# CrystalAnalyst/Lsm

Measured on AMD Instinct MI355X. Metric: GiB/s device-resident SSTable block encode+decode, 4 KiB blocks, 1/2/4/8 GPU, higher is better.
Workload: dtype u8; 1 GPU; U: 1048576 blocks/GPU x block_size 4096, decode + re-encode (16-B uniform keys, 100-B values); blocks_per_gpu=1048576, entries_per_gpu=32474205, encoded_bytes_per_gpu=4226189427, decoded_bytes_per_gpu=4286595060, block_size=4096, segments_per_gpu=2045, parallelism=block-sharded x1 (no data-path collective), encode_output=segments packed (lsmblk_encode_batch), rccl_world=1

## Files before the change

### lsm_amd/csrc/lsmblk_gpu.hip

```cpp
#include "lsmblk_dev.hpp"

namespace {


struct DecodeArgs {
  const uint8_t* blocks;
  const uint64_t* blk_off;
  uint64_t nblk;
  uint8_t* keys;
  uint32_t* key_off;
  uint8_t* vals;
  uint32_t* val_off;
  uint64_t* ts;
  uint64_t entry_cap, key_cap, val_cap;
  uint64_t* stats;
  const uint32_t* agg;
  const uint64_t* tile_pre;
  uint32_t tail;
  uint64_t* blk_ent;
  uint32_t skip;
  uint64_t* bagg;
  uint64_t* bbase;
  uint64_t* tagg;
  uint64_t* tinc;
  uint64_t lag;
  uint64_t lag_bytes;
  uint64_t* dbg;
  uint32_t tag, poll;
};

constexpr uint32_t kTile = 64;
constexpr uint32_t kDbgTiles = 32768, kDbgWords = 16 + 8 * kDbgTiles;
__device__ __forceinline__ void dbg_trace(uint64_t* dbg, uint64_t t, uint32_t k) {
  if (kDiag && dbg && t < kDbgTiles && lane_id() == 0) dbg[16 + 8 * t + k] = __builtin_amdgcn_s_memrealtime();
}


constexpr uint32_t kLB = 2;
#ifndef LSMBLK_XEB
#define LSMBLK_XEB 4
#endif
constexpr uint32_t kEB = LSMBLK_XEB;
constexpr uint32_t kEBBlock = 2;


constexpr uint32_t kDecImg = 4128;
constexpr uint32_t kDecMaxE = 128;
constexpr uint32_t kDecOut = 4032;

struct alignas(16) DecLds {
  uint8_t img[kDecImg];
  alignas(16) uint8_t out[kDecOut];
};
static_assert(sizeof(DecLds) == 8160, "decode LDS: 20 blocks per CU");

struct DecTables {
  uint16_t epos[kDecMaxE], pfx[kDecMaxE], sfx[kDecMaxE];
  uint32_t kout[kDecMaxE + 1], vout[kDecMaxE + 1];
};
static_assert(sizeof(DecTables) <= kDecImg, "large-block tables overlay the image");

struct DecEnt {
  uint32_t epos, p, s, kout, vout, vl;
};

__device__ __forceinline__ void lds_read16(const uint8_t* base, uint32_t x, uint32_t (&v)[4]) {
  const u32x4 q = *reinterpret_cast<const u32x4*>(base + x);
  v[0] = q.x, v[1] = q.y, v[2] = q.z, v[3] = q.w;
}

constexpr int kLdAux = 0;

template <class Img>
__device__ void dec_simple_outputs(const DecodeArgs& a, const Img& im, const BlockHdr& h,
                                   uint64_t E0, uint64_t K0, uint64_t V0) {
  const uint32_t l = lane_id();
  uint64_t kc = 0, vc = 0;
  for (uint32_t c = 0; c < h.n; c += 64) {
    const uint32_t k = c + l;
    uint32_t off = 0, p = 0, s = 0, vl = 0;
    if (k < h.n) parse_entry(im, h, k, off, p, s, vl);
    const uint64_t kl = p + s;
    const uint64_t ki = wave_incl_scan<uint64_t>(kl), vi = wave_incl_scan<uint64_t>(vl);
    const uint64_t kpos = K0 + kc + ki - kl, vpos = V0 + vc + vi - vl;
    kc += __shfl(ki, 63, 64);
    vc += __shfl(vi, 63, 64);
    if (k < h.n) {
      const uint64_t e = E0 + k;
      if (e < a.entry_cap) {
        a.ts[e] = im.u64(off + 4 + s);
        a.key_off[e] = uint32_t(kpos);
        a.val_off[e] = uint32_t(vpos);
      }
      for (uint32_t t = 0; t < p; ++t)
        if (kpos + t < a.key_cap) a.keys[kpos + t] = uint8_t(im.u8(4 + t));
      for (uint32_t t = 0; t < s; ++t)
        if (kpos + p + t < a.key_cap) a.keys[kpos + p + t] = uint8_t(im.u8(off + 4 + t));
      for (uint32_t t = 0; t < vl; ++t)
        if (vpos + t < a.val_cap) a.vals[vpos + t] = uint8_t(im.u8(off + 14 + s + t));
    }
  }
}

__device__ __forceinline__ void st16(const rsrc_t& R, uint32_t off, const uint32_t (&v)[4]) {
  const u32x4 q = {v[0], v[1], v[2], v[3]};
  __builtin_amdgcn_raw_buffer_store_b128(q, R, off, 0, 0);
}

__device__ __forceinline__ void st_short(const rsrc_t& R, uint32_t off, uint32_t len, const uint32_t (&v)[4]) {
  if (len >= 8) {
    __builtin_amdgcn_raw_buffer_store_b64(u32x2{v[0], v[1]}, R, off, 0, 0);
    const uint32_t x = len - 8, sh = x & 3;
    const uint32_t w0 = x < 4 ? v[0] : v[1], w1 = x < 4 ? v[1] : v[2], w2 = x < 4 ? v[2] : v[3];
    __builtin_amdgcn_raw_buffer_store_b64(
        u32x2{__builtin_amdgcn_alignbyte(w1, w0, sh), __builtin_amdgcn_alignbyte(w2, w1, sh)}, R, off + x, 0, 0);
  } else if (len >= 4) {
    __builtin_amdgcn_raw_buffer_store_b32(v[0], R, off, 0, 0);
    __builtin_amdgcn_raw_buffer_store_b32(__builtin_amdgcn_alignbyte(v[1], v[0], len - 4), R, off + len - 4, 0, 0);
  } else {
    for (uint32_t i = 0; i < len; ++i)
      __builtin_amdgcn_raw_buffer_store_b8(uint8_t(v[0] >> (8 * i)), R, off + i, 0, 0);
  }
}

struct GlbSink {
  rsrc_t RK, RV;
  uint32_t kb, vb;
  __device__ __forceinline__ void put16(bool val, uint32_t off, const uint32_t (&v)[4]) const {
    st16(val ? RV : RK, (val ? vb : kb) + off, v);
  }
  __device__ __forceinline__ void put_short(bool val, uint32_t off, uint32_t len, const uint32_t (&v)[4]) const {
    st_short(val ? RV : RK, (val ? vb : kb) + off, len, v);
  }
};
struct LdsSink {
  uint8_t* out;
  uint32_t kb, vb;
  __device__ __forceinline__ void put16(bool val, uint32_t off, const uint32_t (&v)[4]) const {
    *reinterpret_cast<u32x4*>(out + (val ? vb : kb) + off) = u32x4{v[0], v[1], v[2], v[3]};
  }
  __device__ __forceinline__ void put_short(bool val, uint32_t off, uint32_t len, const uint32_t (&v)[4]) const {
    uint8_t* p = out + (val ? vb : kb) + off;
    if (len >= 8) {
      const uint32_t x = len - 8, sh = x & 3;
      const uint32_t w0 = x < 4 ? v[0] : v[1], w1 = x < 4 ? v[1] : v[2], w2 = x < 4 ? v[2] : v[3];
      *reinterpret_cast<u32x2*>(p) = u32x2{v[0], v[1]};
      *reinterpret_cast<u32x2*>(p + x) =
          u32x2{__builtin_amdgcn_alignbyte(w1, w0, sh), __builtin_amdgcn_alignbyte(w2, w1, sh)};
    } else if (len >= 4) {
      *reinterpret_cast<uint32_t*>(p) = v[0];
      *reinterpret_cast<uint32_t*>(p + len - 4) = __builtin_amdgcn_alignbyte(v[1], v[0], len - 4);
    } else {
      for (uint32_t i = 0; i < len; ++i) p[i] = uint8_t(v[0] >> (8 * i));
    }
  }
};

#ifndef LSMBLK_XDEC_VALN
#define LSMBLK_XDEC_VALN 1
#endif
template <class Sink>
__device__ __forceinline__ void dec_entry_runs(const DecodeArgs& a, DecLds& L, uint32_t lead, uint32_t n,
                                               const DecEnt (&ent)[2], uint64_t E0, uint64_t K0, uint64_t V0,
                                               const Sink& out, uint32_t skip) {
  const uint32_t l = lane_id();
  const uint8_t* img = L.img;
  const uint32_t fk = lead + 4;
#pragma unroll
  for (uint32_t it = 0; it < 2; ++it) {
    if (64 * it >= n) break;
    const uint32_t k = 64 * it + l;
    const bool live = k < n;
    const uint32_t epos = ent[it].epos, p = ent[it].p, s = ent[it].s;
    const uint32_t kout = ent[it].kout, vout = ent[it].vout, vl = ent[it].vl;
    const uint32_t sb = lead + epos + 4;
    const uint32_t kl = p + s;
    const bool kirr = live && (kl < 16 || sb < p);
    const bool kuni = !__ballot(kirr);
    const uint32_t nkmax = __builtin_amdgcn_readlane(wave_incl_max32(live ? (kl + 15) >> 4 : 0u), 63);
    const uint32_t nvmax = __builtin_amdgcn_readlane(wave_incl_max32(live && vl >= 16 ? (vl + 15) >> 4 : 0u), 63);
    const uint32_t vS = sb + s + 10, vD = out.vb + vout;
    bool valn = false;
    uint32_t vm = 0, vmmax = 0, vS1 = 0, vD1 = 0;
    if constexpr (std::is_same_v<Sink, LdsSink>) {
      valn = LSMBLK_XDEC_VALN && it == 0 && n <= 64 && !__ballot(live && (vl < 16 || (l == 0 && vS < (vD & 15)))) &&
             !(skip & (4 | 32 | 64));
      if (valn) {
        const uint32_t cs = l == 0 ? (vD >> 4) : ((vD + 15) >> 4), ce = (vD + vl - 1) >> 4;
        vm = live ? ce - cs + 1 : 0u;
        vmmax = __builtin_amdgcn_readlane(wave_incl_max32(vm), 63);
        vS1 = uint32_t(__shfl(int(vS), int(min(l + 1, 63u)), 64));
        vD1 = uint32_t(__shfl(int(vD), int(min(l + 1, 63u)), 64));
      }
    }
    if (!live) continue;
    if (!(skip & 8)) {
      const uint64_t e = E0 + k;
      const u32x2 q = LSMBLK_XALIGNED_LDS ? lds_qw_al(img, sb + s) : *reinterpret_cast<const u32x2*>(img + sb + s);
      a.ts[e] = __builtin_bswap64((uint64_t(q.y) << 32) | q.x);
      a.key_off[e] = uint32_t(K0 + kout);
      a.val_off[e] = uint32_t(V0 + vout);
    }
    if (!(skip & 2)) {
      auto merged = [&](uint32_t o, uint32_t (&v)[4]) {
        const u32x4 sq = *reinterpret_cast<const u32x4*>(img + sb + o - p);
        const u32x4 fq = *reinterpret_cast<const u32x4*>(img + fk + o);
        const uint32_t sv[4] = {sq.x, sq.y, sq.z, sq.w}, fv[4] = {fq.x, fq.y, fq.z, fq.w};
#pragma unroll
        for (uint32_t d = 0; d < 4; ++d) {
          const int32_t nf = int32_t(p) - int32_t(o + 4 * d);
          const uint32_t m = nf <= 0 ? 0u : nf >= 4 ? ~0u : (1u << (8 * nf)) - 1;
          v[d] = (fv[d] & m) | (sv[d] & ~m);
        }
      };
      if (kuni) {
        for (uint32_t t = 0; t < nkmax; ++t) {
          const uint32_t o = min(16 * t, kl - 16);
          uint32_t v[4];
          merged(o, v);
          out.put16(false, kout + o, v);
        }
      } else {
        for (uint32_t t = 0; t < kl; t += 16) {
          const uint32_t o = kl >= 16 ? min(t, kl - 16) : 0u;
          uint32_t v[4];
          if (sb + o >= p) {
            merged(o, v);
          } else {
#pragma unroll
            for (uint32_t d = 0; d < 4; ++d) {
              uint32_t wd = 0;
              for (uint32_t i = 0; i < 4; ++i) {
                const uint32_t x = o + 4 * d + i;
                wd |= uint32_t(x < p ? img[fk + x] : img[sb + x - p]) << (8 * i);
              }
              v[d] = wd;
            }
          }
          if (kl >= 16) out.put16(false, kout + o, v);
          else out.put_short(false, kout, kl, v);
        }
      }
    }
    if (valn) {
      uint8_t* const ob = L.out;
      auto funnel = [](const uint32_t (&d)[6], uint32_t x, uint32_t (&v)[4]) {
        const uint32_t m = (x & 4) ? ~0u : 0u;
        uint32_t y[5];
#pragma unroll
        for (uint32_t j = 0; j < 5; ++j) y[j] = __builtin_amdgcn_bitop3_b32(m, d[j + 1], d[j], 0xCA);
#pragma unroll
        for (uint32_t i = 0; i < 4; ++i) v[i] = __builtin_amdgcn_alignbyte(y[i + 1], y[i], x & 3);
      };
      auto rd8 = [&](uint32_t x, uint32_t& lo, uint32_t& hi) {
        const u32x2 q = *reinterpret_cast<const u32x2*>(img + x);
        lo = q.x, hi = q.y;
      };
      const uint32_t cs = l == 0 ? (vD >> 4) : ((vD + 15) >> 4);
      const uint32_t a0 = vS + 16 * cs - vD;
      uint32_t d[6], x8 = a0 & ~7u;
      rd8(x8, d[0], d[1]);
      rd8(x8 + 8, d[2], d[3]);
      rd8(x8 + 16, d[4], d[5]);
      for (uint32_t i = 0; i < vmmax; ++i) {
        if (i < vm) {
          uint32_t v[4];
          funnel(d, a0, v);
          const uint32_t c = cs + i, cut = vD + vl - 16 * c;
          if (cut < 16 && k + 1 < n) {
            const uint32_t a1 = vS1 + 16 * c - vD1, y8 = a1 & ~7u;
            uint32_t e[6], w[4];
            rd8(y8, e[0], e[1]);
            rd8(y8 + 8, e[2], e[3]);
            rd8(y8 + 16, e[4], e[5]);
            funnel(e, a1, w);
#pragma unroll
            for (uint32_t q = 0; q < 4; ++q) {
              const int32_t nb = int32_t(cut) - int32_t(4 * q);
              const uint32_t msk = nb <= 0 ? 0u : nb >= 4 ? ~0u : (1u << (8 * nb)) - 1;
              v[q] = (v[q] & msk) | (w[q] & ~msk);
            }
          }
          *reinterpret_cast<u32x4*>(ob + 16 * c) = u32x4{v[0], v[1], v[2], v[3]};
          d[0] = d[4], d[1] = d[5];
          x8 += 16;
          rd8(x8 + 8, d[2], d[3]);
          rd8(x8 + 16, d[4], d[5]);
        }
      }
    } else if (!(skip & 4)) {
      const uint32_t src = sb + s + 10;
      if (vl >= 16) {
        for (uint32_t i0 = 0; i0 < nvmax; i0 += kLB) {
          u32x4 q[kLB];
          uint32_t o[kLB];
          const uint32_t am = (skip & 32) ? 15u : (skip & 64) ? 3u : 0u;
#pragma unroll
          for (uint32_t j = 0; j < kLB; ++j) {
            o[j] = min(16 * (i0 + j), vl - 16);
            q[j] = *reinterpret_cast<const u32x4*>(img + ((src + o[j]) & ~am));
          }
#pragma unroll
          for (uint32_t j = 0; j < kLB; ++j) {
            const uint32_t v[4] = {q[j].x, q[j].y, q[j].z, q[j].w};
            const uint32_t xa = (out.vb + vout + o[j]) & ~am;
            out.put16(true, xa >= out.vb ? xa - out.vb : xa + am + 1 - out.vb, v);
          }
        }
      } else if (vl) {
        const u32x4 q = *reinterpret_cast<const u32x4*>(img + src);
        const uint32_t v[4] = {q.x, q.y, q.z, q.w};
        out.put_short(true, vout, vl, v);
      }
    }
  }
}

template <uint32_t B = kLB>
__device__ __forceinline__ void flush_run(uint8_t* gdst_aligned, const uint8_t* lds, uint32_t lo, uint32_t len) {
  flush_chunks<B, LSMBLK_XDEC_STORE>(gdst_aligned, lds, lo, len, lane_id(), 64);
}

template <uint32_t B>
__device__ __forceinline__ void flush_run_masked(uint8_t* gdst_aligned, const uint8_t* lds, uint32_t lo, uint32_t len) {
  const uint32_t end = lo + len, nc = (end + 15) >> 4;
  const uint32_t l = lane_id();
  for (uint32_t c0 = 0; c0 < nc; c0 += 64 * B) {
    u32x4 q[B];
#pragma unroll
    for (uint32_t j = 0; j < B; ++j) {
      const uint32_t c = c0 + 64 * j + l;
      if (c < nc) q[j] = *reinterpret_cast<const u32x4*>(lds + 16 * c);
    }
#pragma unroll
    for (uint32_t j = 0; j < B; ++j) {
      const uint32_t c = c0 + 64 * j + l;
      if (c < nc) {
        const uint32_t v[4] = {q[j].x, q[j].y, q[j].z, q[j].w};
        const uint32_t a0 = 16 * c < lo ? lo - 16 * c : 0u;
        const uint32_t a1 = min(end - 16 * c, 16u);
        store_chunk(gdst_aligned + 16 * c, v, a0, a1);
      }
    }
  }
}

__device__ void dec_fast_outputs(const DecodeArgs& a, DecLds& L, uint32_t lead, const BlockHdr& h,
                                 const DecEnt (&ent)[2], uint64_t E0, uint64_t K0, uint64_t V0, uint32_t K,
                                 uint32_t V, uint32_t skip) {
  const uint32_t kb = uint32_t(K0 & 15), vb = uint32_t(V0 & 15);
  const uint32_t vrun = (kb + K + 15) & ~15u;
  if (vrun + ((vb + V + 15) & ~15u) <= kDecOut) {
    dec_entry_runs(a, L, lead, h.n, ent, E0, K0, V0, LdsSink{L.out, kb, vrun + vb}, skip);
    wave_sync();
    flush_run(a.keys + (K0 - kb), L.out, kb, K);
    flush_run(a.vals + (V0 - vb), L.out + vrun, vb, V);
  } else {
    const GlbSink g{make_rsrc_exact(a.keys + (K0 - kb), kb + K), make_rsrc_exact(a.vals + (V0 - vb), vb + V), kb, vb};
    dec_entry_runs(a, L, lead, h.n, ent, E0, K0, V0, g, skip);
  }
}

constexpr uint32_t kBigB = 8;

__device__ __forceinline__ u32x4 gload16(const rsrc_t& R, uint32_t off) {
  return __builtin_amdgcn_raw_buffer_load_b128(R, off, 0, 0);
}

__device__ __forceinline__ void copy_run(const rsrc_t& RS, uint32_t so, uint32_t lim, const rsrc_t& RD, uint32_t dof,
                                         uint32_t len) {
  if (len == 0) return;
  if (len < 16) {
    uint32_t v[4] = {0, 0, 0, 0};
    if (so + 16 <= lim) {
      const u32x4 q = gload16(RS, so);
      v[0] = q.x, v[1] = q.y, v[2] = q.z, v[3] = q.w;
    } else {
      for (uint32_t i = 0; i < len; ++i) v[i >> 2] |= __builtin_amdgcn_raw_buffer_load_b8(RS, so + i, 0, 0) << (8 * (i & 3));
    }
    st_short(RD, dof, len, v);
    return;
  }
  const uint32_t np = (len + 15) >> 4, last = len - 16;
  for (uint32_t j0 = 0; j0 < np; j0 += kBigB) {
    u32x4 q[kBigB];
#pragma unroll
    for (uint32_t j = 0; j < kBigB; ++j)
      if (j0 + j < np) q[j] = gload16(RS, so + min(16 * (j0 + j), last));
#pragma unroll
    for (uint32_t j = 0; j < kBigB; ++j)
      if (j0 + j < np) {
        const uint32_t v[4] = {q[j].x, q[j].y, q[j].z, q[j].w};
        st16(RD, dof + min(16 * (j0 + j), last), v);
      }
  }
}

__device__ __forceinline__ void copy_run1(const rsrc_t& RS, uint32_t so, uint32_t lim, const rsrc_t& RD, uint32_t dof,
                                          uint32_t len) {
  if (len < 16) {
    copy_run(RS, so, lim, RD, dof, len);
    return;
  }
  const uint32_t last = len - 16;
  for (uint32_t o = 0;; o += 16) {
    const uint32_t x = min(o, last);
    const u32x4 q = gload16(RS, so + x);
    const uint32_t v[4] = {q.x, q.y, q.z, q.w};
    st16(RD, dof + x, v);
    if (x == last) break;
  }
}

constexpr uint32_t kCoop = 16;
__device__ __forceinline__ void copy_run_wave(const rsrc_t& RS, uint32_t so, const rsrc_t& RD, uint32_t dof,
                                              uint32_t len) {
  const uint32_t l = lane_id();
  const uint32_t np = (len + 15) >> 4, last = len - 16;
  for (uint32_t j0 = 0; j0 < np; j0 += 64 * kBigB) {
    u32x4 q[kBigB];
#pragma unroll
    for (uint32_t j = 0; j < kBigB; ++j) {
      const uint32_t idx = j0 + 64 * j + l;
      if (idx < np) q[j] = gload16(RS, so + min(16 * idx, last));
    }
#pragma unroll
    for (uint32_t j = 0; j < kBigB; ++j) {
      const uint32_t idx = j0 + 64 * j + l;
      if (idx < np) {
        const uint32_t v[4] = {q[j].x, q[j].y, q[j].z, q[j].w};
        st16(RD, dof + min(16 * idx, last), v);
      }
    }
  }
}

constexpr uint32_t kCopyScratch = 4 * 64 + 64;
static_assert(4 * kCopyScratch <= kDecOut, "the decode's large-block path lends its output image");

template <uint32_t B>
struct CopyBatch {
  u32x4 q[B];
  uint32_t dst[B];
};

template <uint32_t B>
__device__ __forceinline__ void copy_issue(const rsrc_t& RS, uint32_t g0, uint32_t total, uint32_t np, uint32_t first,
                                           uint32_t* sc, uint32_t& carry, CopyBatch<B>& c) {
  const uint32_t l = lane_id();
  const u32x4* rec = reinterpret_cast<const u32x4*>(sc);
  uint32_t* mark = sc + 4 * 64;
  uint32_t own[B];
#pragma unroll
  for (uint32_t j = 0; j < B; ++j) {
    const uint32_t G = g0 + 64 * j;
    own[j] = 0;
    if (G < total) {
      mark[l] = 0;
      wave_sync();
      if (np != 0 && first - G < 64u) mark[first - G] = l + 1;
      wave_sync();
      const uint32_t m = max(wave_incl_max32(mark[l]), carry);
      carry = __builtin_amdgcn_readlane(m, 63);
      own[j] = m - 1;
      wave_sync();
    }
  }
#pragma unroll
  for (uint32_t j = 0; j < B; ++j) {
    const uint32_t g = g0 + 64 * j + l;
    c.dst[j] = ~0u;
    if (g < total) {
      const u32x4 r = rec[own[j]];
      const uint32_t off = min(16 * (g - r.w), r.z);
      c.q[j] = gload16(RS, r.x + off);
      c.dst[j] = r.y + off;
    }
  }
}

template <uint32_t B>
__device__ __forceinline__ void copy_store(const rsrc_t& RD, const CopyBatch<B>& c) {
#pragma unroll
  for (uint32_t j = 0; j < B; ++j)
    if (c.dst[j] != ~0u) {
      const uint32_t v[4] = {c.q[j].x, c.q[j].y, c.q[j].z, c.q[j].w};
      st16(RD, c.dst[j], v);
    }
}

struct NoAfter {
  __device__ void operator()(uint32_t, uint32_t, uint32_t) const {}
};
template <uint32_t B = kBigB, class After = NoAfter>
__device__ __forceinline__ void copy_long_runs(bool longrun, const rsrc_t& RS, uint32_t so, const rsrc_t& RD,
                                               uint32_t dof, uint32_t len, uint32_t* sc, const After& after = After()) {
  const uint32_t l = lane_id();
  const uint32_t np = longrun ? (len + 15) >> 4 : 0u;
  const uint32_t incl = wave_incl_scan32(np);
  const uint32_t total = __builtin_amdgcn_readlane(incl, 63);
  const uint32_t first = incl - np;
  if (total == 0) {
    after(first, 0u, ~0u);
    return;
  }
  wave_sync();
  reinterpret_cast<u32x4*>(sc)[l] = u32x4{so, dof, len - 16, first};
  uint32_t carry = 0;
  for (uint32_t g0 = 0; g0 < total; g0 += 64 * B) {
    CopyBatch<B> c;
    copy_issue(RS, g0, total, np, first, sc, carry, c);
    copy_store(RD, c);
    after(first, g0, g0 + 64 * B >= total ? ~0u : g0 + 64 * B);
  }
}

__device__ __forceinline__ void dec_big_entry(const DecodeArgs& a, const DecTables& L, const GlbImg& im, uint32_t k,
                                              uint32_t lim, const rsrc_t& RK, uint32_t kb, uint64_t E0, uint64_t K0,
                                              uint64_t V0) {
  const rsrc_t& R = im.r;
  const uint32_t lead = im.lead, fk = lead + 4;
  const uint32_t epos = L.epos[k], p = L.pfx[k], s = L.sfx[k], kout = L.kout[k];
  const uint32_t sb = lead + epos + 4, kl = p + s;
  const uint64_t e = E0 + k;
  a.ts[e] = im.u64(epos + 4 + s);
  a.key_off[e] = uint32_t(K0 + kout);
  a.val_off[e] = uint32_t(V0 + L.vout[k]);
  for (uint32_t t = 0; t < kl; t += 16) {
    const uint32_t o = kl >= 16 ? min(t, kl - 16) : 0u;
    uint32_t v[4];
    if (sb + o >= p && sb + o - p + 16 <= lim && fk + o + 16 <= lim) {
      const u32x4 sq = gload16(R, sb + o - p), fq = gload16(R, fk + o);
      const uint32_t sv[4] = {sq.x, sq.y, sq.z, sq.w}, fv[4] = {fq.x, fq.y, fq.z, fq.w};
#pragma unroll
      for (uint32_t d = 0; d < 4; ++d) {
        const int32_t nf = int32_t(p) - int32_t(o + 4 * d);
        const uint32_t m = nf <= 0 ? 0u : nf >= 4 ? ~0u : (1u << (8 * nf)) - 1;
        v[d] = (fv[d] & m) | (sv[d] & ~m);
      }
    } else {
#pragma unroll
      for (uint32_t d = 0; d < 4; ++d) {
        uint32_t wd = 0;
        for (uint32_t i = 0; i < 4; ++i) {
          const uint32_t x = o + 4 * d + i;
          wd |= (x < p ? im.u8(4 + x) : im.u8(epos + 4 + x - p)) << (8 * i);
        }
        v[d] = wd;
      }
    }
    if (kl >= 16) st16(RK, kb + kout + o, v);
    else st_short(RK, kb + kout, kl, v);
  }
}

#ifndef LSMBLK_XDBB
#define LSMBLK_XDBB 8
#endif
constexpr uint32_t kDecBigB = LSMBLK_XDBB;

__device__ void dec_big_outputs(const DecodeArgs& a, const DecTables& L, const rsrc_t& R, uint32_t lead,
                                const BlockHdr& h, uint32_t n, uint64_t Eb, uint64_t K0, uint64_t V0, uint32_t K,
                                uint32_t V, uint32_t* sc) {
  const uint32_t l = lane_id();
  const uint32_t kb = uint32_t(K0 & 15), vb = uint32_t(V0 & 15);
  const rsrc_t RK = make_rsrc_exact(a.keys + (K0 - kb), kb + K), RV = make_rsrc_exact(a.vals + (V0 - vb), vb + V);
  const GlbImg im{R, lead};
  const uint32_t lim = lead + h.len;
  for (uint32_t c = 0; c < n; c += 64) {
    const uint32_t k = c + l;
    const bool live = k < n;
    uint32_t vsrc = 0, vdst = 0, vl = 0;
    if (live) {
      dec_big_entry(a, L, im, k, lim, RK, kb, Eb, K0, V0);
      vsrc = lead + L.epos[k] + 14 + L.sfx[k];
      vdst = vb + L.vout[k];
      vl = L.vout[k + 1] - L.vout[k];
      if (vl < kCoop) copy_run(R, vsrc, lim, RV, vdst, vl);
    }
    copy_long_runs<kDecBigB>(live && vl >= kCoop, R, vsrc, RV, vdst, vl, sc);
  }
}

template <bool lagm, class Mid, class Post, class PreWait>
__device__ void decode_block(const DecodeArgs& a, DecLds& L, uint64_t b, uint64_t start, uint64_t end, Mid&& mid,
                             Post&& post, PreWait&& pre_wait) {
  const uint32_t l = lane_id();
  uint32_t err = 0;
  const uint64_t tb = b / kTile, jb = b % kTile;
  uint32_t cn = 0, ck = 0, cv = 0;
  uint64_t tp0 = 0, tp1 = 0, tp2 = 0, gb = 0;
  if constexpr (!lagm) {
    if (l < jb) {
      const uint64_t q = tb * kTile + l;
      cn = a.agg[3 * q];
      ck = a.agg[3 * q + 1];
      cv = a.agg[3 * q + 2];
    }
    tp0 = a.tile_pre[3 * tb], tp1 = a.tile_pre[3 * tb + 1], tp2 = a.tile_pre[3 * tb + 2];
  }
  uint32_t len = 0;
  if (end < start + a.tail || end - start > 0x7FFFFFF0ull) err |= LSMBLK_ERR_MALFORMED;
  else len = uint32_t(end - start) - a.tail;
  const uint8_t* bp = a.blocks + start;
  const uint32_t lead = uni(uint32_t(reinterpret_cast<uintptr_t>(bp) & 15));
  const uint8_t* abase = bp - lead;
  const rsrc_t R = make_rsrc(abase, lead + len);
  const bool fits = lead + len + 15 <= kDecImg;

  BlockHdr h;
  if (fits) {
    const uint32_t nchunk = (lead + len + 15) >> 4;
    u32x4 v[5];
    if constexpr (lagm) {
      const uint32_t o = 16 * l, o4 = o + 4096;
      asm volatile(
          "s_nop 4\n\t"
          "buffer_load_dwordx4 %0, %5, %7, 0 offen\n\t"
          "buffer_load_dwordx4 %1, %5, %7, 0 offen offset:1024\n\t"
          "buffer_load_dwordx4 %2, %5, %7, 0 offen offset:2048\n\t"
          "buffer_load_dwordx4 %3, %5, %7, 0 offen offset:3072\n\t"
          "buffer_load_dwordx4 %4, %6, %7, 0 offen"
          : "=&v"(v[0]), "=&v"(v[1]), "=&v"(v[2]), "=&v"(v[3]), "=&v"(v[4])
          : "v"(o), "v"(o4), "s"(R));
      mid();
      asm volatile("s_waitcnt vmcnt(0)" ::: "memory");
#pragma unroll
      for (uint32_t i = 0; i < 5; ++i) asm volatile("" : "+v"(v[i]));
    } else {
#pragma unroll
      for (uint32_t i = 0; i < 5; ++i)
        v[i] = __builtin_amdgcn_raw_buffer_load_b128(R, (l + 64 * i) * 16, 0, kLdAux);
    }
// ... 75 lines not shown
      V += wave_sum<uint64_t>(vl);
    }
  }
  if (diag_mask(a.skip) & 512) return;
  if (__ballot(bad)) err |= LSMBLK_ERR_MALFORMED;
  uint64_t agg[3] = {h.n, K, V};
  if (err) agg[0] = agg[1] = agg[2] = 0;

  pre_wait();
  uint64_t excl[3];
  if constexpr (lagm) {
    const uint64_t want = (uint64_t(a.tag) << 2) | 2;
    uint32_t spins = 0;
    if (b % kTile == 0) dbg_trace(a.dbg, b / kTile, 2);
    while (!(diag_mask(a.skip) & 2048) && __ballot(l < 3 && (gb & 0xFFFF) != want)) {
      if (++spins > kSpinLimit) {
        err |= LSMBLK_ERR_TIMEOUT;
        break;
      }
      __builtin_amdgcn_s_sleep(1);
      if (l < 3 && (gb & 0xFFFF) != want) gb = gload(a.bbase + 3 * b + l, a.poll);
    }
#pragma unroll
    for (uint32_t q = 0; q < 3; ++q)
      excl[q] = uint64_t(uint32_t(__builtin_amdgcn_readlane(uint32_t(gb >> 16), q))) |
                (uint64_t(uint32_t(__builtin_amdgcn_readlane(uint32_t(gb >> 48), q))) << 32);
    if (b % kTile == 0) dbg_trace(a.dbg, b / kTile, 3);
  } else {
    excl[0] = tp0 + wave_sum(cn);
    excl[1] = tp1 + wave_sum(ck);
    excl[2] = tp2 + wave_sum(cv);
  }
  wave_sync();
  const uint64_t E0 = excl[0], K0 = excl[1], V0 = excl[2];
  if (a.blk_ent && l == 0) a.blk_ent[b] = E0;
  const uint64_t Et = E0 + agg[0], Kt = K0 + agg[1], Vt = V0 + agg[2];
  if (Kt > 0xFFFFFFFFull || Vt > 0xFFFFFFFFull) err |= LSMBLK_ERR_OVERFLOW;
  if (Et > a.entry_cap || Kt > a.key_cap || Vt > a.val_cap) err |= LSMBLK_ERR_CAPACITY;
  if (lagm && b + 1 == a.nblk && l == 0) {
    if (a.blk_ent) a.blk_ent[a.nblk] = Et;
    a.stats[0] = Et;
    a.stats[1] = Kt;
    a.stats[2] = Vt;
    if (Et <= a.entry_cap) {
      a.key_off[Et] = uint32_t(Kt);
      a.val_off[Et] = uint32_t(Vt);
    }
  }

  if (!(err & (LSMBLK_ERR_MALFORMED | LSMBLK_ERR_TIMEOUT | LSMBLK_ERR_OVERFLOW | LSMBLK_ERR_CAPACITY)) && h.n) {
    if (fast) {
      dec_fast_outputs(a, L, lead, h, ent, E0, K0, V0, uint32_t(K), uint32_t(V), diag_mask(a.skip));
    } else if (big && h.n <= kDecMaxE) {
      dec_big_outputs(a, T, R, lead, h, h.n, E0, K0, V0, uint32_t(K), uint32_t(V), reinterpret_cast<uint32_t*>(L.out));
    } else if (big) {
      uint64_t kr = 0, vr = 0;
      for (uint32_t c0 = 0; c0 < h.n; c0 += kDecMaxE) {
        const uint32_t nc = min(kDecMaxE, h.n - c0);
        wave_sync();
        parse_tables(GlbImg{R, lead}, c0, nc, kr, vr);
        wave_sync();
        dec_big_outputs(a, T, R, lead, h, nc, E0 + c0, K0, V0, uint32_t(K), uint32_t(V), reinterpret_cast<uint32_t*>(L.out));
      }
    } else if (fits) {
      dec_simple_outputs(a, LdsImg{L.img, lead}, h, E0, K0, V0);
    } else {
      dec_simple_outputs(a, GlbImg{R, lead}, h, E0, K0, V0);
    }
  }
  raise_err(a.stats, err);
}

__global__ __launch_bounds__(64) void decode_kernel(DecodeArgs a) {
  __shared__ DecLds lds;
  const uint64_t b = blockIdx.x;
  decode_block<false>(a, lds, b, uni64(a.blk_off[b]), uni64(a.blk_off[b + 1]), [] {}, [] {}, [] {});
}


__device__ __forceinline__ uint64_t sat47(uint64_t v) { return v > (1ull << 47) - 1 ? (1ull << 47) - 1 : v; }

__device__ __forceinline__ void publish3(uint64_t* arr, uint64_t idx, uint64_t x0, uint64_t x1, uint64_t x2,
                                         uint32_t tag, uint32_t flag, uint32_t poll) {
  const uint32_t l = lane_id();
  const uint64_t x = l == 0 ? x0 : (l == 1 ? x1 : x2);
  if (l < 3) gstore(arr + 3 * idx + l, (sat47(x) << 16) | (uint64_t(tag) << 2) | flag, poll);
}

struct BlkCount {
  uint32_t n;
  uint64_t K, V;
  bool bad;
};
struct CntPre {
  rsrc_t R;
  uint32_t len, lead;
  bool ok, staged;
  u32x4 v[5];
};
__device__ __forceinline__ CntPre cnt_issue(const uint8_t* blocks, uint32_t tail, uint64_t start, uint64_t end) {
  const uint32_t l = lane_id();
  CntPre C;
  C.ok = !(end < start + tail || end - start > 0x7FFFFFF0ull);
  C.len = C.ok ? uint32_t(end - start) - tail : 0u;
  const uint8_t* bp = blocks + start;
  C.lead = uni(uint32_t(reinterpret_cast<uintptr_t>(bp) & 15));
  C.R = make_rsrc(bp - C.lead, C.lead + C.len);
  C.staged = C.ok && C.lead + C.len + 15 <= kDecImg;
  if (C.staged) {
#pragma unroll
    for (uint32_t i = 0; i < 5; ++i)
      C.v[i] = __builtin_amdgcn_raw_buffer_load_b128(C.R, (l + 64 * i) * 16, 0, kLdAux);
  }
  return C;
}
__device__ __forceinline__ BlkCount cnt_finish(const CntPre& C, uint8_t* img) {
  const uint32_t l = lane_id();
  BlkCount r{0, 0, 0, false};
  bool bad = false;
  auto count = [&](const auto& im) {
    const BlockHdr h = parse_hdr(im, C.len);
    if (!h.ok) {
      bad = true;
      return;
    }
    r.n = h.n;
// ... 60 lines not shown
  const FinPf f0 = pf ? *pf : fin_prefetch(a, t);
  uint64_t g0 = f0.g0, g1 = f0.g1, g2 = f0.g2;
  uint32_t spins = 0;
  for (;;) {
    const bool here = (g0 & 0xFFFF) == want && (g1 & 0xFFFF) == want && (g2 & 0xFFFF) == want;
    if (!__ballot(!here)) break;
    if (++spins > kSpinLimit) {
      err |= LSMBLK_ERR_TIMEOUT;
      return;
    }
    __builtin_amdgcn_s_sleep(1);
    if (!here) {
      g0 = gload(a.bagg + 3 * (b0 + l), a.poll);
      g1 = gload(a.bagg + 3 * (b0 + l) + 1, a.poll);
      g2 = gload(a.bagg + 3 * (b0 + l) + 2, a.poll);
    }
  }
  const uint64_t x0 = mine ? g0 >> 16 : 0, x1 = mine ? g1 >> 16 : 0, x2 = mine ? g2 >> 16 : 0;
  const uint64_t i0 = wave_incl_scan<uint64_t>(x0), i1 = wave_incl_scan<uint64_t>(x1), i2 = wave_incl_scan<uint64_t>(x2);
  const uint64_t A[3] = {lane64(i0, 63), lane64(i1, 63), lane64(i2, 63)};
  uint64_t X[3] = {0, 0, 0};
  if (t == 0) {
    publish3(a.tinc, t, A[0], A[1], A[2], a.tag, 2, a.poll);
  } else {
    publish3(a.tagg, t, A[0], A[1], A[2], a.tag, 1, a.poll);
    const uint64_t wi = (uint64_t(a.tag) << 2) | 2;
    uint64_t g = wi;
    if (l < 3) g = gload(a.tinc + 3 * (t - 1) + l, 0);
    if (!__ballot(l < 3 && (g & 0xFFFF) != wi)) {
#pragma unroll
      for (uint32_t q = 0; q < 3; ++q)
        X[q] = uint64_t(uint32_t(__builtin_amdgcn_readlane(uint32_t(g >> 16), q))) |
               (uint64_t(uint32_t(__builtin_amdgcn_readlane(uint32_t(g >> 48), q))) << 32);
    } else {
      if (!lookback<3>(a.tagg, a.tinc, t, a.tag, a.poll, X)) {
        err |= LSMBLK_ERR_TIMEOUT;
        return;
      }
    }
    publish3(a.tinc, t, X[0] + A[0], X[1] + A[1], X[2] + A[2], a.tag, 2, a.poll);
  }
  if (mine) {
    const uint64_t tg = (uint64_t(a.tag) << 2) | 2;
    gstore(a.bbase + 3 * (b0 + l), (sat47(X[0] + i0 - x0) << 16) | tg, a.poll);
    gstore(a.bbase + 3 * (b0 + l) + 1, (sat47(X[1] + i1 - x1) << 16) | tg, a.poll);
    gstore(a.bbase + 3 * (b0 + l) + 2, (sat47(X[2] + i2 - x2) << 16) | tg, a.poll);
  }
  if (kDiag && a.dbg) {
    asm volatile("s_waitcnt vmcnt(0)" ::: "memory");
    dbg_trace(a.dbg, t, 1);
  }
}

__global__ __launch_bounds__(64) void decode_lag_kernel(DecodeArgs a) {
  __shared__ DecLds lds;
  const uint32_t j = blockIdx.x, nblk = uint32_t(a.nblk), lag0 = uint32_t(a.lag);
  const bool cnt = j < nblk;
  const uint32_t l = lane_id();
  uint64_t o = 0;
  if ((l < 2 && cnt) || (l >= 2 && l < 4 && j >= lag0)) o = a.blk_off[(l < 2 ? j : j - lag0) + (l & 1)];
  const uint64_t o0 = a.lag_bytes ? a.blk_off[0] : 0, o1 = a.lag_bytes ? a.blk_off[nblk] : 0;
  const uint64_t cs = lane64(o, 0), ce = lane64(o, 1);
  CntPre C;
  const bool do_cnt = cnt && !(diag_mask(a.skip) & 1024);
  if (do_cnt) C = cnt_issue(a.blocks, a.tail, cs, ce);
  uint32_t lag = lag0;
  if (a.lag_bytes) {
    const uint32_t tot = uint32_t(min((o1 - o0) >> 12, uint64_t(0xFFFFFFFFu))), lb = uint32_t(a.lag_bytes >> 12);
    if (uint64_t(lb) * nblk < uint64_t(lag) * tot) {
      const uint32_t want = uint32_t(float(lb) * (float(nblk) / float(tot)));
      lag = want < 2 * kTile ? 2 * kTile : want;
    }
  }
  if (j >= nblk + lag) return;
  const bool dec = j >= lag;
  if (j % kTile == 0) dbg_trace(a.dbg, j / kTile, 4);
  if (dec && (j - lag) % kTile == 0) dbg_trace(a.dbg, (j - lag) / kTile, 5);
  const uint32_t b = j - lag;
  if (lag != lag0 && dec && l >= 2 && l < 4) o = a.blk_off[b + (l & 1)];
  const uint64_t ds = lane64(o, 2), de = lane64(o, 3);
  uint32_t err = 0;
  BlkCount r{0, 0, 0, false};
  auto count = [&] {
    if (!do_cnt) return;
    r = cnt_finish(C, lds.img);
    wave_sync();
  };
  const uint32_t D = lag / 2 + 63;
  const uint32_t ft = j >= D ? (j - D + 8) / kTile : ~0u;
  const bool fin = j >= D && ft * kTile + D - (ft & 7) == j && ft * kTile < nblk;
  auto publish = [&] {
    if (!cnt || (diag_mask(a.skip) & 16384)) return;
    publish3(a.bagg, j, r.n, r.K, r.V, a.tag, 1, a.poll);
    if (r.K > 0xFFFFFFFFull || r.V > 0xFFFFFFFFull) err |= LSMBLK_ERR_OVERFLOW;
  };
  FinPf fpf{};
  if (fin) fpf = fin_prefetch(a, ft);
  auto finish = [&] {
    if (fin && !(diag_mask(a.skip) & (8192 | 16384))) lag_tile_finish(a, ft, err, &fpf);
  };
  if (dec) {
    decode_block<true>(a, lds, b, ds, de, count, publish, finish);
  } else {
    count();
    publish();
    finish();
  }
// ... 684 lines not shown
  uint32_t skip;
  const uint64_t* dn;
};

__device__ __forceinline__ EmitArgs resolve(const EmitArgs& a0) {
  EmitArgs a = a0;
  if (a.dn) a.n = uni64(*a.dn);
  return a;
}

constexpr uint32_t kEmitWaves = 4;
constexpr uint32_t kEmitKCap = 1088;
constexpr uint32_t kEmitICap = 4224;
constexpr uint32_t kEmitMaxE = 128;
constexpr uint32_t kEmitModeDefault = 2;
constexpr uint64_t kEmitGridMax = 1ull << 18;

struct alignas(16) EmitLds {
  uint8_t kimg[kEmitKCap];
  uint8_t img[kEmitICap];
  alignas(16) uint32_t cent[kEmitICap / 16 + 4];
  alignas(16) uint32_t erec[4 * kEmitMaxE];
  uint64_t ts[kEmitMaxE];
};
struct alignas(16) EmitBlockLds {
  uint8_t kimg[kEmitKCap];
  uint8_t img[kEmitICap];
  alignas(16) uint32_t cent[kEmitICap / 16 + 4];
};
static_assert(sizeof(EmitBlockLds) <= 8192, "at least 20 single-wave workgroups per CU");
struct EmitRecLds {};
struct EmitRecReg {
  uint32_t x[2], y[2], z[2];
  uint64_t ts[2];
};
__device__ __forceinline__ void rec_put_ts(EmitLds& L, EmitRecLds&, uint32_t, uint32_t k, uint64_t v) { L.ts[k] = v; }
__device__ __forceinline__ void rec_put_ts(EmitBlockLds&, EmitRecReg& R, uint32_t it, uint32_t, uint64_t v) { R.ts[it] = v; }
__device__ __forceinline__ uint64_t rec_ts(const EmitLds& L, const EmitRecLds&, uint32_t, uint32_t k) { return L.ts[k]; }
__device__ __forceinline__ uint64_t rec_ts(const EmitBlockLds&, const EmitRecReg& R, uint32_t it, uint32_t) { return R.ts[it]; }
__device__ __forceinline__ void rec_put(EmitLds& L, EmitRecLds&, uint32_t, uint32_t k, uint32_t x, uint32_t y, uint32_t z) {
  *reinterpret_cast<u32x4*>(L.erec + 4 * k) = u32x4{x, y, z, 0u};
}
__device__ __forceinline__ void rec_put(EmitBlockLds&, EmitRecReg& R, uint32_t it, uint32_t, uint32_t x, uint32_t y, uint32_t z) {
  R.x[it] = x, R.y[it] = y, R.z[it] = z;
}
__device__ __forceinline__ u32x4 rec_get(const EmitLds& L, const EmitRecLds&, uint32_t, uint32_t k) {
  return *reinterpret_cast<const u32x4*>(L.erec + 4 * k);
}
__device__ __forceinline__ u32x4 rec_get(const EmitBlockLds&, const EmitRecReg& R, uint32_t it, uint32_t) {
  return u32x4{R.x[it], R.y[it], R.z[it], 0u};
}
__device__ __forceinline__ uint32_t rec_pos(const EmitLds& L, const EmitRecLds&, uint32_t, uint32_t k) { return L.erec[4 * k] & 0xFFFF; }
__device__ __forceinline__ uint32_t rec_pos(const EmitBlockLds&, const EmitRecReg& R, uint32_t it, uint32_t) { return R.x[it] & 0xFFFF; }

__device__ __forceinline__ void lds_st_short(uint8_t* p, uint32_t len, const uint32_t (&v)[4]) {
  if (len >= 8) {
    const uint32_t x = len - 8, sh = x & 3;
    const uint32_t w0 = x < 4 ? v[0] : v[1], w1 = x < 4 ? v[1] : v[2], w2 = x < 4 ? v[2] : v[3];
    *reinterpret_cast<u32x2*>(p) = u32x2{v[0], v[1]};
    *reinterpret_cast<u32x2*>(p + x) = u32x2{__builtin_amdgcn_alignbyte(w1, w0, sh), __builtin_amdgcn_alignbyte(w2, w1, sh)};
  } else if (len >= 4) {
    *reinterpret_cast<uint32_t*>(p) = v[0];
    *reinterpret_cast<uint32_t*>(p + len - 4) = __builtin_amdgcn_alignbyte(v[1], v[0], len - 4);
  } else {
    for (uint32_t i = 0; i < len; ++i) p[i] = uint8_t(v[0] >> (8 * i));
  }
}

#ifndef LSMBLK_XEBB
#define LSMBLK_XEBB 4
#endif
constexpr uint32_t kEmitBigB = LSMBLK_XEBB;

struct BigBlk {
  uint64_t bi, O, size;
  uint32_t s, n;
};
struct BigL1 {
  uint32_t ko0, ko1, vo0, vo1;
};
struct BigL2 {
  u32x4 own, first;
};

struct EmitMeta {
  uint64_t bi;
  uint32_t s, e, n;
  uint64_t O, size;
  uint32_t kb0, kb1, vb0, vb1;
  bool bad;
};

constexpr uint64_t kPlanFatal =
    LSMBLK_ERR_SEGMENTS | LSMBLK_ERR_TIMEOUT | LSMBLK_ERR_INTERNAL | LSMBLK_ERR_EMPTY_KEY | LSMBLK_ERR_MALFORMED;

struct EmitBlk {
  uint32_t s, n;
  uint64_t O, size;
  uint32_t kb0, vb0, klead, vlead, olead, fl, kb1, vb1;
};
struct EmitPf {
  uint32_t ko0 = 0, ko1 = 0, vo0 = 0, vo1 = 0;
  uint64_t ts = 0;
};

#define EAL(x, m) ((diag_mask(a.skip) & 1u) ? ((x) & ~uint32_t(m)) : (x))
template <bool kChk, class Lds, class Rec>
__device__ __forceinline__ uint32_t emit_phase1(const EmitArgs& a, Lds& L, Rec& R, const EmitBlk& B, const EmitPf& pf,
                                                uint32_t (&eh)[2][4], uint32_t (&et)[2][4], uint32_t& ncs, uint32_t& err) {
  const uint32_t l = lane_id();
  const uint32_t s = B.s, n = B.n, kb0 = B.kb0, vb0 = B.vb0, klead = B.klead, vlead = B.vlead, olead = B.olead, fl = B.fl;
  const uint64_t size = B.size;
  ncs = (olead + uint32_t(size) + 15) >> 4;
  for (uint32_t j = 4 * l; j < ncs; j += 256) *reinterpret_cast<u32x4*>(L.cent + j) = u32x4{~0u, ~0u, ~0u, ~0u};
  uint32_t fkw[4];
#pragma unroll
  for (int i = 0; i < 4; ++i) fkw[i] = lds_dword_at(L.kimg, klead + 4 * i);
  uint32_t dc = 0;
#pragma unroll
  for (uint32_t it = 0; it < 2; ++it) {
// ... 2365 lines not shown
```

Measured before the change: 1028 GiB/s.

## Compact decoded values in place in the block image via a chunk map

```diff
diff --git a/lsm_amd/csrc/lsmblk_gpu.hip b/lsm_amd/csrc/lsmblk_gpu.hip
--- a/lsm_amd/csrc/lsmblk_gpu.hip
+++ b/lsm_amd/csrc/lsmblk_gpu.hip
@@ -37,6 +37,7 @@
 
 
 constexpr uint32_t kLB = 2;
+constexpr uint32_t kDecMB = 2;
 #ifndef LSMBLK_XEB
 #define LSMBLK_XEB 4
 #endif
@@ -46,13 +47,17 @@
 
 constexpr uint32_t kDecImg = 4128;
 constexpr uint32_t kDecMaxE = 128;
+constexpr uint32_t kDecKeyImg = 2176;
+constexpr uint32_t kDecMapN = 256;
 constexpr uint32_t kDecOut = 4032;
+static_assert(kDecOut <= 16 * kDecMapN && 16 * kDecMapN <= kDecImg, "the chunk map covers the value run");
 
 struct alignas(16) DecLds {
   uint8_t img[kDecImg];
-  alignas(16) uint8_t out[kDecOut];
+  alignas(16) uint8_t kimg[kDecKeyImg];
+  alignas(16) uint16_t cmap[kDecMapN];
 };
-static_assert(sizeof(DecLds) == 8160, "decode LDS: 20 blocks per CU");
+static_assert(sizeof(DecLds) <= (160 << 10) / 24, "decode LDS: room for 24 blocks per CU");
 
 struct DecTables {
   uint16_t epos[kDecMaxE], pfx[kDecMaxE], sfx[kDecMaxE];
@@ -123,6 +128,20 @@
   }
 }
 
+__device__ __forceinline__ void lds_st_short(uint8_t* p, uint32_t len, const uint32_t (&v)[4]) {
+  if (len >= 8) {
+    const uint32_t x = len - 8, sh = x & 3;
+    const uint32_t w0 = x < 4 ? v[0] : v[1], w1 = x < 4 ? v[1] : v[2], w2 = x < 4 ? v[2] : v[3];
+    *reinterpret_cast<u32x2*>(p) = u32x2{v[0], v[1]};
+    *reinterpret_cast<u32x2*>(p + x) = u32x2{__builtin_amdgcn_alignbyte(w1, w0, sh), __builtin_amdgcn_alignbyte(w2, w1, sh)};
+  } else if (len >= 4) {
+    *reinterpret_cast<uint32_t*>(p) = v[0];
+    *reinterpret_cast<uint32_t*>(p + len - 4) = __builtin_amdgcn_alignbyte(v[1], v[0], len - 4);
+  } else {
+    for (uint32_t i = 0; i < len; ++i) p[i] = uint8_t(v[0] >> (8 * i));
+  }
+}
+
 struct GlbSink {
   rsrc_t RK, RV;
   uint32_t kb, vb;
@@ -134,35 +153,23 @@
   }
 };
 struct LdsSink {
-  uint8_t* out;
-  uint32_t kb, vb;
-  __device__ __forceinline__ void put16(bool val, uint32_t off, const uint32_t (&v)[4]) const {
-    *reinterpret_cast<u32x4*>(out + (val ? vb : kb) + off) = u32x4{v[0], v[1], v[2], v[3]};
-  }
-  __device__ __forceinline__ void put_short(bool val, uint32_t off, uint32_t len, const uint32_t (&v)[4]) const {
-    uint8_t* p = out + (val ? vb : kb) + off;
-    if (len >= 8) {
-      const uint32_t x = len - 8, sh = x & 3;
-      const uint32_t w0 = x < 4 ? v[0] : v[1], w1 = x < 4 ? v[1] : v[2], w2 = x < 4 ? v[2] : v[3];
-      *reinterpret_cast<u32x2*>(p) = u32x2{v[0], v[1]};
-      *reinterpret_cast<u32x2*>(p + x) =
-          u32x2{__builtin_amdgcn_alignbyte(w1, w0, sh), __builtin_amdgcn_alignbyte(w2, w1, sh)};
-    } else if (len >= 4) {
-      *reinterpret_cast<uint32_t*>(p) = v[0];
-      *reinterpret_cast<uint32_t*>(p + len - 4) = __builtin_amdgcn_alignbyte(v[1], v[0], len - 4);
-    } else {
-      for (uint32_t i = 0; i < len; ++i) p[i] = uint8_t(v[0] >> (8 * i));
-    }
+  uint8_t* kimg;
+  uint32_t kb;
+  uint16_t* cmap;
+  uint32_t vb;
+  __device__ __forceinline__ void put16(bool, uint32_t off, const uint32_t (&v)[4]) const {
+    *reinterpret_cast<u32x4*>(kimg + kb + off) = u32x4{v[0], v[1], v[2], v[3]};
+  }
+  __device__ __forceinline__ void put_short(bool, uint32_t off, uint32_t len, const uint32_t (&v)[4]) const {
+    lds_st_short(kimg + kb + off, len, v);
   }
 };
 
-#ifndef LSMBLK_XDEC_VALN
-#define LSMBLK_XDEC_VALN 1
-#endif
 template <class Sink>
 __device__ __forceinline__ void dec_entry_runs(const DecodeArgs& a, DecLds& L, uint32_t lead, uint32_t n,
                                                const DecEnt (&ent)[2], uint64_t E0, uint64_t K0, uint64_t V0,
-                                               const Sink& out, uint32_t skip) {
+                                               const Sink& out, uint32_t skip, uint32_t (&eh)[2][4],
+                                               uint32_t (&et)[2][4]) {
   const uint32_t l = lane_id();
   const uint8_t* img = L.img;
   const uint32_t fk = lead + 4;
@@ -178,21 +185,9 @@
     const bool kirr = live && (kl < 16 || sb < p);
     const bool kuni = !__ballot(kirr);
     const uint32_t nkmax = __builtin_amdgcn_readlane(wave_incl_max32(live ? (kl + 15) >> 4 : 0u), 63);
-    const uint32_t nvmax = __builtin_amdgcn_readlane(wave_incl_max32(live && vl >= 16 ? (vl + 15) >> 4 : 0u), 63);
-    const uint32_t vS = sb + s + 10, vD = out.vb + vout;
-    bool valn = false;
-    uint32_t vm = 0, vmmax = 0, vS1 = 0, vD1 = 0;
-    if constexpr (std::is_same_v<Sink, LdsSink>) {
-      valn = LSMBLK_XDEC_VALN && it == 0 && n <= 64 && !__ballot(live && (vl < 16 || (l == 0 && vS < (vD & 15)))) &&
-             !(skip & (4 | 32 | 64));
-      if (valn) {
-        const uint32_t cs = l == 0 ? (vD >> 4) : ((vD + 15) >> 4), ce = (vD + vl - 1) >> 4;
-        vm = live ? ce - cs + 1 : 0u;
-        vmmax = __builtin_amdgcn_readlane(wave_incl_max32(vm), 63);
-        vS1 = uint32_t(__shfl(int(vS), int(min(l + 1, 63u)), 64));
-        vD1 = uint32_t(__shfl(int(vD), int(min(l + 1, 63u)), 64));
-      }
-    }
+    uint32_t nvmax = 0;
+    if constexpr (!std::is_same_v<Sink, LdsSink>)
+      nvmax = __builtin_amdgcn_readlane(wave_incl_max32(live && vl >= 16 ? (vl + 15) >> 4 : 0u), 63);
     if (!live) continue;
     if (!(skip & 8)) {
       const uint64_t e = E0 + k;
@@ -242,54 +237,16 @@
         }
       }
     }
-    if (valn) {
-      uint8_t* const ob = L.out;
-      auto funnel = [](const uint32_t (&d)[6], uint32_t x, uint32_t (&v)[4]) {
-        const uint32_t m = (x & 4) ? ~0u : 0u;
-        uint32_t y[5];
-#pragma unroll
-        for (uint32_t j = 0; j < 5; ++j) y[j] = __builtin_amdgcn_bitop3_b32(m, d[j + 1], d[j], 0xCA);
-#pragma unroll
-        for (uint32_t i = 0; i < 4; ++i) v[i] = __builtin_amdgcn_alignbyte(y[i + 1], y[i], x & 3);
-      };
-      auto rd8 = [&](uint32_t x, uint32_t& lo, uint32_t& hi) {
-        const u32x2 q = *reinterpret_cast<const u32x2*>(img + x);
-        lo = q.x, hi = q.y;
-      };
-      const uint32_t cs = l == 0 ? (vD >> 4) : ((vD + 15) >> 4);
-      const uint32_t a0 = vS + 16 * cs - vD;
-      uint32_t d[6], x8 = a0 & ~7u;
-      rd8(x8, d[0], d[1]);
-      rd8(x8 + 8, d[2], d[3]);
-      rd8(x8 + 16, d[4], d[5]);
-      for (uint32_t i = 0; i < vmmax; ++i) {
-        if (i < vm) {
-          uint32_t v[4];
-          funnel(d, a0, v);
-          const uint32_t c = cs + i, cut = vD + vl - 16 * c;
-          if (cut < 16 && k + 1 < n) {
-            const uint32_t a1 = vS1 + 16 * c - vD1, y8 = a1 & ~7u;
-            uint32_t e[6], w[4];
-            rd8(y8, e[0], e[1]);
-            rd8(y8 + 8, e[2], e[3]);
-            rd8(y8 + 16, e[4], e[5]);
-            funnel(e, a1, w);
-#pragma unroll
-            for (uint32_t q = 0; q < 4; ++q) {
-              const int32_t nb = int32_t(cut) - int32_t(4 * q);
-              const uint32_t msk = nb <= 0 ? 0u : nb >= 4 ? ~0u : (1u << (8 * nb)) - 1;
-              v[q] = (v[q] & msk) | (w[q] & ~msk);
-            }
-          }
-          *reinterpret_cast<u32x4*>(ob + 16 * c) = u32x4{v[0], v[1], v[2], v[3]};
-          d[0] = d[4], d[1] = d[5];
-          x8 += 16;
-          rd8(x8 + 8, d[2], d[3]);
-          rd8(x8 + 16, d[4], d[5]);
-        }
+    const uint32_t src = sb + s + 10;
+    if constexpr (std::is_same_v<Sink, LdsSink>) {
+      if (vl && !(skip & 4)) {
+        lds_read16(img, src, eh[it]);
+        lds_read16(img, src + (vl > 16 ? vl - 16 : 0u), et[it]);
+        const uint32_t vD = out.vb + vout;
+        const uint32_t d = src - vD;
+        for (uint32_t c = (vD + 15) >> 4; 16 * c + 16 <= vD + vl; ++c) out.cmap[c] = uint16_t(d + 16 * c);
       }
     } else if (!(skip & 4)) {
-      const uint32_t src = sb + s + 10;
       if (vl >= 16) {
         for (uint32_t i0 = 0; i0 < nvmax; i0 += kLB) {
           u32x4 q[kLB];
@@ -348,16 +305,67 @@
 __device__ void dec_fast_outputs(const DecodeArgs& a, DecLds& L, uint32_t lead, const BlockHdr& h,
                                  const DecEnt (&ent)[2], uint64_t E0, uint64_t K0, uint64_t V0, uint32_t K,
                                  uint32_t V, uint32_t skip) {
+  const uint32_t l = lane_id();
+  const uint32_t n = h.n;
   const uint32_t kb = uint32_t(K0 & 15), vb = uint32_t(V0 & 15);
-  const uint32_t vrun = (kb + K + 15) & ~15u;
-  if (vrun + ((vb + V + 15) & ~15u) <= kDecOut) {
-    dec_entry_runs(a, L, lead, h.n, ent, E0, K0, V0, LdsSink{L.out, kb, vrun + vb}, skip);
+  int32_t dprev = 0;
+  bool mono = true;
+#pragma unroll
+  for (uint32_t it = 0; it < 2; ++it) {
+    if (64 * it >= n) break;
+    const bool live = 64 * it + l < n;
+    const int32_t d = live ? int32_t(lead + ent[it].epos + 14 + ent[it].s) - int32_t(vb + ent[it].vout) : 0x7FFFFFFF;
+    const int32_t up = __shfl_up(d, 1, 64);
+    mono = mono && d >= (l ? up : dprev);
+    dprev = __builtin_amdgcn_readlane(d, 63);
+  }
+  const uint32_t krun = (kb + K + 15) & ~15u;
+  if (!__ballot(!mono) && krun <= kDecKeyImg && krun + ((vb + V + 15) & ~15u) <= kDecOut) {
+    static_assert(sizeof(DecLds::cmap) == 32 * 16, "the map is zeroed by 32 lanes");
+    if (l < 32) reinterpret_cast<u32x4*>(L.cmap)[l] = u32x4{0, 0, 0, 0};
     wave_sync();
-    flush_run(a.keys + (K0 - kb), L.out, kb, K);
-    flush_run(a.vals + (V0 - vb), L.out + vrun, vb, V);
+    uint32_t eh[2][4] = {}, et[2][4] = {};
+    dec_entry_runs(a, L, lead, n, ent, E0, K0, V0, LdsSink{L.kimg, kb, L.cmap, vb}, skip, eh, et);
+    wave_sync();
+    flush_run(a.keys + (K0 - kb), L.kimg, kb, K);
+    if (!(skip & 4)) {
+      const uint32_t nw = (vb + V) >> 4;
+      for (uint32_t c0 = 0; c0 < nw; c0 += 64 * kDecMB) {
+        uint32_t src[kDecMB] = {};
+        u32x4 v[kDecMB] = {};
+#pragma unroll
+        for (uint32_t j = 0; j < kDecMB; ++j) {
+          const uint32_t c = c0 + 64 * j + l;
+          src[j] = c < nw ? L.cmap[c] : 0u;
+        }
+#pragma unroll
+        for (uint32_t j = 0; j < kDecMB; ++j)
+          if (src[j]) v[j] = *reinterpret_cast<const u32x4*>(L.img + src[j]);
+#pragma unroll
+        for (uint32_t j = 0; j < kDecMB; ++j)
+          if (src[j]) *reinterpret_cast<u32x4*>(L.img + 16 * (c0 + 64 * j + l)) = v[j];
+      }
+      wave_sync();
+#pragma unroll
+      for (uint32_t it = 0; it < 2; ++it) {
+        if (64 * it >= n) break;
+        const uint32_t vl = ent[it].vl;
+        uint8_t* const o = L.img + vb + ent[it].vout;
+        if (64 * it + l >= n) continue;
+        if (vl >= 16) {
+          *reinterpret_cast<u32x4*>(o) = u32x4{eh[it][0], eh[it][1], eh[it][2], eh[it][3]};
+          *reinterpret_cast<u32x4*>(o + vl - 16) = u32x4{et[it][0], et[it][1], et[it][2], et[it][3]};
+        } else if (vl) {
+          lds_st_short(o, vl, eh[it]);
+        }
+      }
+      wave_sync();
+      flush_run(a.vals + (V0 - vb), L.img, vb, V);
+    }
   } else {
     const GlbSink g{make_rsrc_exact(a.keys + (K0 - kb), kb + K), make_rsrc_exact(a.vals + (V0 - vb), vb + V), kb, vb};
-    dec_entry_runs(a, L, lead, h.n, ent, E0, K0, V0, g, skip);
+    uint32_t eh[2][4], et[2][4];
+    dec_entry_runs(a, L, lead, n, ent, E0, K0, V0, g, skip, eh, et);
   }
 }
 
@@ -436,7 +444,7 @@
 }
 
 constexpr uint32_t kCopyScratch = 4 * 64 + 64;
-static_assert(4 * kCopyScratch <= kDecOut, "the decode's large-block path lends its output image");
+static_assert(4 * kCopyScratch <= kDecKeyImg, "the decode's large-block path lends its key image");
 
 template <uint32_t B>
 struct CopyBatch {
@@ -444,10 +452,14 @@
   uint32_t dst[B];
 };
 
-template <uint32_t B>
+template <uint32_t B, bool PIN = false>
 __device__ __forceinline__ void copy_issue(const rsrc_t& RS, uint32_t g0, uint32_t total, uint32_t np, uint32_t first,
                                            uint32_t* sc, uint32_t& carry, CopyBatch<B>& c) {
   const uint32_t l = lane_id();
+  if constexpr (PIN) {
+#pragma unroll
+    for (uint32_t j = 0; j < B; ++j) asm volatile("" : "=v"(c.q[j]));
+  }
   const u32x4* rec = reinterpret_cast<const u32x4*>(sc);
   uint32_t* mark = sc + 4 * 64;
   uint32_t own[B];
@@ -473,10 +485,23 @@
     if (g < total) {
       const u32x4 r = rec[own[j]];
       const uint32_t off = min(16 * (g - r.w), r.z);
-      c.q[j] = gload16(RS, r.x + off);
+      const uint32_t src = r.x + off;
+      if constexpr (PIN) {
+        if (j == 0) asm volatile("s_nop 4\n\tbuffer_load_dwordx4 %0, %1, %2, 0 offen" : "+v"(c.q[j]) : "v"(src), "s"(RS));
+        else asm volatile("buffer_load_dwordx4 %0, %1, %2, 0 offen" : "+v"(c.q[j]) : "v"(src), "s"(RS));
+      } else {
+        c.q[j] = gload16(RS, src);
+      }
       c.dst[j] = r.y + off;
     }
   }
+}
+
+template <uint32_t B>
+__device__ __forceinline__ void copy_land(CopyBatch<B>& c) {
+  asm volatile("s_waitcnt vmcnt(0)" ::: "memory");
+#pragma unroll
+  for (uint32_t j = 0; j < B; ++j) asm volatile("" : "+v"(c.q[j]));
 }
 
 template <uint32_t B>
@@ -492,7 +517,7 @@
 struct NoAfter {
   __device__ void operator()(uint32_t, uint32_t, uint32_t) const {}
 };
-template <uint32_t B = kBigB, class After = NoAfter>
+template <uint32_t B = kBigB, bool PIN = false, class After = NoAfter>
 __device__ __forceinline__ void copy_long_runs(bool longrun, const rsrc_t& RS, uint32_t so, const rsrc_t& RD,
                                                uint32_t dof, uint32_t len, uint32_t* sc, const After& after = After()) {
   const uint32_t l = lane_id();
@@ -509,7 +534,8 @@
   uint32_t carry = 0;
   for (uint32_t g0 = 0; g0 < total; g0 += 64 * B) {
     CopyBatch<B> c;
-    copy_issue(RS, g0, total, np, first, sc, carry, c);
+    copy_issue<B, PIN>(RS, g0, total, np, first, sc, carry, c);
+    if constexpr (PIN) copy_land(c);
     copy_store(RD, c);
     after(first, g0, g0 + 64 * B >= total ? ~0u : g0 + 64 * B);
   }
@@ -578,7 +604,7 @@
       vl = L.vout[k + 1] - L.vout[k];
       if (vl < kCoop) copy_run(R, vsrc, lim, RV, vdst, vl);
     }
-    copy_long_runs<kDecBigB>(live && vl >= kCoop, R, vsrc, RV, vdst, vl, sc);
+    copy_long_runs<kDecBigB, true>(live && vl >= kCoop, R, vsrc, RV, vdst, vl, sc);
   }
 }
 
@@ -760,7 +786,7 @@
     if (fast) {
       dec_fast_outputs(a, L, lead, h, ent, E0, K0, V0, uint32_t(K), uint32_t(V), diag_mask(a.skip));
     } else if (big && h.n <= kDecMaxE) {
-      dec_big_outputs(a, T, R, lead, h, h.n, E0, K0, V0, uint32_t(K), uint32_t(V), reinterpret_cast<uint32_t*>(L.out));
+      dec_big_outputs(a, T, R, lead, h, h.n, E0, K0, V0, uint32_t(K), uint32_t(V), reinterpret_cast<uint32_t*>(L.kimg));
     } else if (big) {
       uint64_t kr = 0, vr = 0;
       for (uint32_t c0 = 0; c0 < h.n; c0 += kDecMaxE) {
@@ -768,7 +794,7 @@
         wave_sync();
         parse_tables(GlbImg{R, lead}, c0, nc, kr, vr);
         wave_sync();
-        dec_big_outputs(a, T, R, lead, h, nc, E0 + c0, K0, V0, uint32_t(K), uint32_t(V), reinterpret_cast<uint32_t*>(L.out));
+        dec_big_outputs(a, T, R, lead, h, nc, E0 + c0, K0, V0, uint32_t(K), uint32_t(V), reinterpret_cast<uint32_t*>(L.kimg));
       }
     } else if (fits) {
       dec_simple_outputs(a, LdsImg{L.img, lead}, h, E0, K0, V0);
@@ -779,7 +805,7 @@
   raise_err(a.stats, err);
 }
 
-__global__ __launch_bounds__(64) void decode_kernel(DecodeArgs a) {
+__global__ __launch_bounds__(64) __attribute__((amdgpu_waves_per_eu(5))) void decode_kernel(DecodeArgs a) {
   __shared__ DecLds lds;
   const uint64_t b = blockIdx.x;
   decode_block<false>(a, lds, b, uni64(a.blk_off[b]), uni64(a.blk_off[b + 1]), [] {}, [] {}, [] {});
@@ -946,7 +972,7 @@
   }
 }
 
-__global__ __launch_bounds__(64) void decode_lag_kernel(DecodeArgs a) {
+__global__ __launch_bounds__(64) __attribute__((amdgpu_waves_per_eu(5))) void decode_lag_kernel(DecodeArgs a) {
   __shared__ DecLds lds;
   const uint32_t j = blockIdx.x, nblk = uint32_t(a.nblk), lag0 = uint32_t(a.lag);
   const bool cnt = j < nblk;
@@ -1737,20 +1763,6 @@
 }
 __device__ __forceinline__ uint32_t rec_pos(const EmitLds& L, const EmitRecLds&, uint32_t, uint32_t k) { return L.erec[4 * k] & 0xFFFF; }
 __device__ __forceinline__ uint32_t rec_pos(const EmitBlockLds&, const EmitRecReg& R, uint32_t it, uint32_t) { return R.x[it] & 0xFFFF; }
-
-__device__ __forceinline__ void lds_st_short(uint8_t* p, uint32_t len, const uint32_t (&v)[4]) {
-  if (len >= 8) {
-    const uint32_t x = len - 8, sh = x & 3;
-    const uint32_t w0 = x < 4 ? v[0] : v[1], w1 = x < 4 ? v[1] : v[2], w2 = x < 4 ? v[2] : v[3];
-    *reinterpret_cast<u32x2*>(p) = u32x2{v[0], v[1]};
-    *reinterpret_cast<u32x2*>(p + x) = u32x2{__builtin_amdgcn_alignbyte(w1, w0, sh), __builtin_amdgcn_alignbyte(w2, w1, sh)};
-  } else if (len >= 4) {
-    *reinterpret_cast<uint32_t*>(p) = v[0];
-    *reinterpret_cast<uint32_t*>(p + len - 4) = __builtin_amdgcn_alignbyte(v[1], v[0], len - 4);
-  } else {
-    for (uint32_t i = 0; i < len; ++i) p[i] = uint8_t(v[0] >> (8 * i));
-  }
-}
 
 #ifndef LSMBLK_XEBB
 #define LSMBLK_XEBB 4
```

Result: faster. 1041 GiB/s, median of 6 (+1.3%).
